# libvips/libvips

Measured on NVIDIA H100. Metric: Mpixels/s for thumbnail(4K->512,lanczos3), higher is better.
Workload: dtype u8

## Files before the change

### include/vb200.h

```cpp
#ifndef VB200_H
#define VB200_H

#include <stddef.h>
#include <stdint.h>

#ifdef __cplusplus
extern "C" {
#endif


typedef enum {
	VB200_FORMAT_UCHAR = 0,
	VB200_FORMAT_CHAR = 1,
	VB200_FORMAT_USHORT = 2,
	VB200_FORMAT_SHORT = 3,
	VB200_FORMAT_UINT = 4,
	VB200_FORMAT_INT = 5,
	VB200_FORMAT_FLOAT = 6,
	VB200_FORMAT_COMPLEX = 7,
	VB200_FORMAT_DOUBLE = 8,
	VB200_FORMAT_DPCOMPLEX = 9
} VB200BandFormat;

typedef enum {
// ... 135 lines not shown

typedef struct VB200ThumbnailPlan VB200ThumbnailPlan;

VB200ThumbnailPlan *vb200_thumbnail_plan_new(int width, int height, int bands, int band_format, int has_alpha,
	int target_width, int target_height, int size, int linear);
void vb200_thumbnail_plan_free(VB200ThumbnailPlan *plan);
int vb200_thumbnail_plan_output(const VB200ThumbnailPlan *plan, int *out_width, int *out_height);
int vb200_thumbnail_batch_device(VB200ThumbnailPlan *plan, const void *in, size_t in_frame_stride, void *out,
	size_t out_frame_stride, int n_frames);
int vb200_thumbnail_batch_host(VB200ThumbnailPlan *plan, const void *in, size_t in_frame_stride, void *out,
	size_t out_frame_stride, int n_frames);
int vb200_thumbnail_plan_set_sharpen(VB200ThumbnailPlan *plan, double sigma, double x1, double y2, double y3, double m1, double m2);
int vb200_thumbnail_plan_is_fused(const VB200ThumbnailPlan *plan);
size_t vb200_thumbnail_plan_bytes_per_frame(const VB200ThumbnailPlan *plan);
const char *vb200_thumbnail_plan_kernel(const VB200ThumbnailPlan *plan);

typedef struct {
	const void *input_profile;
	size_t input_len;
	const void *output_profile;
	size_t output_len;
	const void *builtin_rgb;
	size_t builtin_rgb_len;
	const void *builtin_grey;
	size_t builtin_grey_len;
	int intent;
} VB200ThumbnailIcc;

int vb200_thumbnail_plan_set_icc(VB200ThumbnailPlan *plan, const VB200ThumbnailIcc *icc);
int vb200_thumbnail_plan_output_bands(const VB200ThumbnailPlan *plan);
// ... 93 lines not shown
```

### libvips_b200/__init__.py

```python
import ctypes as C
import os

import numpy as np

_HERE = os.path.dirname(os.path.abspath(__file__))
_LIB_PATH = os.environ.get("VB200_LIB") or os.path.join(_HERE, "libvb200.so")
_lib = None

HOST, DEVICE = 0, 1

FORMATS = {np.dtype(np.uint8): 0, np.dtype(np.int8): 1, np.dtype(np.uint16): 2, np.dtype(np.int16): 3,
           np.dtype(np.uint32): 4, np.dtype(np.int32): 5, np.dtype(np.float32): 6, np.dtype(np.float64): 8}
DTYPES = {v: k for k, v in FORMATS.items()}
KERNELS = {"nearest": 0, "linear": 1, "cubic": 2, "mitchell": 3, "lanczos2": 4, "lanczos3": 5,
           "mks2013": 6, "mks2021": 7}
SIZES = {"both": 0, "up": 1, "down": 2, "force": 3}
PRECISIONS = {"integer": 0, "float": 1, "approximate": 2}
INTENTS = {"perceptual": 0, "relative": 1, "saturation": 2, "absolute": 3}
PCS = {"lab": 0, "xyz": 1}
INTERPRETATIONS = {"multiband": 0, "b-w": 1, "cmyk": 15, "xyz": 12, "lab": 13, "lch": 19, "labs": 21, "srgb": 22,
                   "yxy": 23, "rgb16": 25, "grey16": 26, "scrgb": 28, "hsv": 29}


class Error(Exception):
# ... 112 lines not shown
                                              C.c_size_t, C.c_size_t, PI, PI, PI]
        L.vb200_debug_jpeg_decode.argtypes = [C.c_void_p, C.c_size_t, C.c_int, C.c_void_p, C.c_size_t, PI, PI, PI]
        L.vb200_thumbnail_jpegshrink.argtypes = [C.c_int] * 5
        L.vb200_jpegsave_batch.argtypes = [C.c_void_p, C.c_int, C.c_size_t, C.c_size_t, C.c_int, C.c_int, C.c_int, C.c_int, C.c_int, C.c_int,
                                           C.c_void_p, C.c_int, C.c_size_t, C.POINTER(C.c_size_t)]
        L.vb200_thumbnail_buffer.argtypes = [C.c_void_p, C.c_size_t, IP, C.c_int, C.c_int, C.c_int]
        L.vb200_thumbnail_plan_run_jpeg.argtypes = [C.c_void_p, C.POINTER(C.c_void_p), C.POINTER(C.c_size_t), C.c_int, C.c_int,
                                                    C.c_void_p, C.c_int, C.c_size_t]
        L.vb200_thumbnail_plan_free.argtypes = [C.c_void_p]
        L.vb200_thumbnail_plan_output.argtypes = [C.c_void_p, C.POINTER(C.c_int), C.POINTER(C.c_int)]
        L.vb200_thumbnail_plan_bytes_per_frame.restype = C.c_size_t
        L.vb200_thumbnail_plan_bytes_per_frame.argtypes = [C.c_void_p]
        L.vb200_thumbnail_plan_is_fused.argtypes = [C.c_void_p]
        L.vb200_thumbnail_plan_kernel.restype = C.c_char_p
        L.vb200_thumbnail_plan_kernel.argtypes = [C.c_void_p]
        L.vb200_thumbnail_batch_device.argtypes = [C.c_void_p, C.c_void_p, C.c_size_t, C.c_void_p, C.c_size_t,
                                                   C.c_int]
        L.vb200_thumbnail_batch_host.argtypes = [C.c_void_p, C.c_void_p, C.c_size_t, C.c_void_p, C.c_size_t,
                                                 C.c_int]
        TI = C.POINTER(CThumbnailIcc)
        L.vb200_thumbnail_plan_set_icc.argtypes = [C.c_void_p, TI]
        L.vb200_thumbnail_plan_output_bands.argtypes = [C.c_void_p]
        L.vb200_thumbnail_batch_device_icc.argtypes = [C.c_void_p, C.c_void_p, C.c_size_t, C.c_void_p, C.c_size_t, C.c_int,
                                                       C.c_void_p, C.c_void_p]
        L.vb200_thumbnail_batch_host_icc.argtypes = L.vb200_thumbnail_batch_device_icc.argtypes
        L.vb200_thumbnail_image_icc.argtypes = [IP, IP, C.c_int, C.c_int, C.c_int, TI, C.c_char_p, C.c_size_t]
        L.vb200_thumbnail_buffer_icc.argtypes = [C.c_void_p, C.c_size_t, IP, C.c_int, C.c_int, C.c_int, TI]
        L.vb200_jpeg_icc_profile.argtypes = [C.c_char_p, C.c_size_t, C.c_void_p, C.c_size_t, C.POINTER(C.c_size_t)]
        L.vb200_debug_icc_select.argtypes = [TI, C.c_int, C.c_char_p, C.c_size_t, C.POINTER(C.c_int)]
        L.vb200_debug_icc_classify.argtypes = [C.c_char_p, C.c_size_t, C.c_int, C.c_int]
# ... 554 lines not shown
```

### libvips_b200/csrc/thumbnail_fused.cu

```cuda
#include <algorithm>
#include <climits>
#include <cmath>
#include <cstring>
#include <map>
#include <memory>
#include <mutex>
#include <vector>

#include <cuda.h>

#include "vb200_internal.h"

namespace vb200 {

namespace {

constexpr int kChunkRows = 8;
constexpr int kMaxThreads = 576;

struct FusedParams {
	int W, H;
	size_t in_bpl;
	int VS;
	int Hs;
// ... 10 lines not shown
	int TW;
	int RPC;
	int NT;
	int NEmax;
	int slots;
	int stage_pitch;
	int vgrid, hgrid;
	const int2 *vrow;
	const int2 *hcol;
	const int *vcoef;
	const int *hcoef;
	int nvsets, nhsets;
	const int2 *vchunk;
	const uint4 *vbfrag;
	int mma_rows;
	int premul;
	const unsigned char *opaque_hint;
	double max_alpha;
};

__device__ __forceinline__ int
dp2a_lo(unsigned coef, unsigned bytes, int acc)
{
	int d;
	asm("dp2a.lo.s32.u32 %0, %1, %2, %3;" : "=r"(d) : "r"(coef), "r"(bytes), "r"(acc));
	return d;
}

__device__ __forceinline__ int
dp2a_hi(unsigned coef, unsigned bytes, int acc)
// ... 1169 lines not shown
	int OW = 0, OH = 0;
	ReduceGeom gv{}, gh{};
	bool premul = false;
	bool fused = false;
	int device = -1;
	FusedParams fp{};
	void *tables = nullptr;
	size_t smem = 0;
	dim3 grid;
	bool tma_ok = false;
	int slots_tma = 0;
	size_t smem_tma = 0;
	bool tma3_ok = false;
	size_t smem_tma3 = 0;
	bool mma_ok = false;
	int mma_cols = 0, mma_cpt = 1, mma_tw = 0, mma_nt = 0, mma_nemax = 0;
	size_t smem_mma = 0;
	void *tables_mma = nullptr;
	static constexpr int kStreams = 3;
	cudaStream_t streams[kStreams] = {nullptr, nullptr, nullptr};
	void *stage_in[kStreams] = {nullptr, nullptr, nullptr};
	void *stage_out[kStreams] = {nullptr, nullptr, nullptr};
	cudaEvent_t drained[kStreams] = {nullptr, nullptr, nullptr};
	int stage_frames = 0;
	std::mutex pump_lock;
	std::mutex launch_lock;
	static constexpr int kHintSlots = 4;
	std::mutex hint_lock;
	int *hint_counts = nullptr;
	cudaEvent_t hint_done[kHintSlots] = {nullptr, nullptr, nullptr, nullptr};
	bool hint_pending[kHintSlots] = {false, false, false, false};
// ... 301 lines not shown
launch_mma_t(const char *domain, ThumbnailPlanImpl *pl, const FusedParams &fp, const void *in, size_t in_stride, void *out,
	size_t out_stride, int n, dim3 grid, cudaStream_t s)
{
	CUtensorMap tm;
	memset(&tm, 0, sizeof(tm));
	const int use_tmap = make_stage_tensor_map(&tm, in, fp.W, fp.H, fp.in_bpl, in_stride, n, (WCOLS + 8) / (WCOLS + 8 > 512 ? 2 : 1), 2 * VS) ? 1 : 0;
	constexpr bool CAN_OPQ = PREMUL && CPT == 2 && WCOLS > 448;
	for (int f0 = 0; f0 < n; f0 += 32768) {
		grid.z = std::min(32768, n - f0);
		FusedParams fpl = fp;
		void *hint = nullptr;
		bool use_opq = false;
		if (CAN_OPQ && opaque_hint_begin(domain, pl, fp, (const uint8_t *) in + (size_t) f0 * in_stride, in_stride, (int) grid.z, s, &hint, &use_opq))
			return -1;
		fpl.opaque_hint = (const unsigned char *) hint;
		int rc;
		if constexpr (CAN_OPQ)
			rc = use_opq ? launch_mma_k<VS, NP, PREMUL, HSQ, WCOLS, CPT, true>(domain, pl, fpl, tm, use_tmap, in, in_stride, out, out_stride, f0, grid, s)
						 : launch_mma_k<VS, NP, PREMUL, HSQ, WCOLS, CPT, false>(domain, pl, fpl, tm, use_tmap, in, in_stride, out, out_stride, f0, grid, s);
		else
			rc = launch_mma_k<VS, NP, PREMUL, HSQ, WCOLS, CPT, false>(domain, pl, fpl, tm, use_tmap, in, in_stride, out, out_stride, f0, grid, s);
		opaque_hint_end(pl, hint, (int) grid.z, s);
		if (rc)
			return rc;
	}
	return 0;
}

template <bool PREMUL, int WCOLS, int CPT>
int
launch_mma_w(const char *domain, ThumbnailPlanImpl *pl, const FusedParams &fp, const void *in, size_t is, void *out,
	size_t os, int n, dim3 grid, cudaStream_t s, bool *handled)
{
	*handled = true;
	const int np = fp.NPh == 6 || fp.NPh == 7 ? fp.NPh : 0;
#define V4(VS_, NP_, HS_) \
	if (fp.VS == VS_ && np == NP_ && fp.HS == HS_) \
// ... 4 lines not shown
	if constexpr (CPT == 2 && WCOLS > 448) {
		V4(3, 0, 3) V4(5, 0, 5) V4(6, 0, 6) V4(7, 0, 7)
		V4(2, 0, 3) V4(3, 0, 2) V4(3, 0, 4) V4(4, 0, 3) V4(4, 0, 5) V4(5, 0, 4) V4(5, 0, 6) V4(6, 0, 5)
		V4(6, 0, 7) V4(7, 0, 6) V4(7, 0, 8) V4(8, 0, 7)
	}
#undef V4
	*handled = false;
	return 0;
}

int
launch_mma(const char *domain, ThumbnailPlanImpl *pl, const void *in, size_t is, void *out, size_t os, int n,
	cudaStream_t s, bool *handled)
{
	FusedParams fp = pl->fp;
	fp.TW = pl->mma_tw;
	fp.NT = pl->mma_nt;
	fp.NEmax = pl->mma_nemax;
	const int K = fp.mma_rows;
	const int bands_x = (pl->OW + fp.TW - 1) / fp.TW;
	int rpc = ((pl->OH + K - 1) / K) * K;
	const int ctas = pl->mma_cols > 448 ? sm_count() : 2 * sm_count();
	while ((long long) bands_x * ((pl->OH + rpc - 1) / rpc) * n < ctas && rpc > 4 * K)
		rpc = ((rpc / 2 + K - 1) / K) * K;
	fp.RPC = rpc;
	const dim3 grid(bands_x, (pl->OH + rpc - 1) / rpc, 1);
	if (pl->mma_cols > 448)
		return pl->premul ? launch_mma_w<true, 768, 2>(domain, pl, fp, in, is, out, os, n, grid, s, handled)
						  : launch_mma_w<false, 768, 2>(domain, pl, fp, in, is, out, os, n, grid, s, handled);
	if (pl->mma_cpt == 1)
		return pl->premul ? launch_mma_w<true, VB200_V4_COLS, 1>(domain, pl, fp, in, is, out, os, n, grid, s, handled)
						  : launch_mma_w<false, VB200_V4_COLS, 1>(domain, pl, fp, in, is, out, os, n, grid, s, handled);
	return pl->premul ? launch_mma_w<true, VB200_V4_COLS, 2>(domain, pl, fp, in, is, out, os, n, grid, s, handled)
					  : launch_mma_w<false, VB200_V4_COLS, 2>(domain, pl, fp, in, is, out, os, n, grid, s, handled);
}
// ... 49 lines not shown
	if (pl->gv.int_shrink > 1) {
		tile_w = tg.tile_width;
		tile_h = tg.tile_height;
	}
	else {
		tile_w = pl->OW;
		tile_h = tg.fatstrip_height;
	}
	int rect_h = tile_h;
	if (pl->gh.int_shrink > 1)
		rect_h = std::min(rect_h, tg.fatstrip_height);
	build_axis_table(tv, pl->OH, pl->gv.residual, pl->gv.offset, pl->gv.n_point, VB200_KERNEL_LANCZOS3, rect_h);
	build_axis_table(th, pl->OW, pl->gh.residual, pl->gh.offset, pl->gh.n_point, VB200_KERNEL_LANCZOS3, tile_w);
}

int
plan_build_fused(const char *domain, ThumbnailPlanImpl *pl)
{
	AxisTable tv, th;
	plan_axis_tables(pl, tv, th);

	auto build_sets = [](const AxisTable &t, int count, int grid, PairSets &sets, std::vector<int2> &idx) {
		sets = PairSets();
		sets.NP = (t.n_point + 2) / 2;
		idx.resize(count);
		for (int i = 0; i < count; i++) {
			const int rel = t.first[i] - grid;
			idx[i].x = rel >> 1;
			idx[i].y = sets.get(t, t.phase[i], rel & 1);
		}
		sets.trim();
	};
	PairSets sv, shh;
	std::vector<int2> vrow, hcol;
	int vgrid = 0, hgrid = 0;
	{
		PairSets alt;
		std::vector<int2> alt_idx;
		build_sets(tv, pl->OH, 0, sv, vrow);
		build_sets(tv, pl->OH, 1, alt, alt_idx);
		if (alt.NP < sv.NP) {
			sv = alt;
			vrow = alt_idx;
			vgrid = 1;
		}
		build_sets(th, pl->OW, 0, shh, hcol);
		build_sets(th, pl->OW, 1, alt, alt_idx);
		if (alt.NP < shh.NP) {
			shh = alt;
			hcol = alt_idx;
			hgrid = 1;
		}
	}

	FusedParams &fp = pl->fp;
	fp.W = pl->W;
	fp.H = pl->H;
	fp.in_bpl = (size_t) pl->W * 4;
	fp.VS = pl->gv.int_shrink;
	fp.Hs = pl->gv.shrunk_size;
	fp.vembed = tv.embed;
	fp.NPv = sv.NP;
	fp.vgrid = vgrid;
	fp.hgrid = hgrid;
	fp.vmul8 = (unsigned) (((1LL << 32) / (256LL * fp.VS)) << 8);
	fp.vshift = -1;
	fp.accmul = 1;
	for (int sft = 0; sft < 9; sft++)
// ... 110 lines not shown
		if (ok) {
			memcpy(vchunk.data(), vchunk_flat.data(), vchunk.size() * sizeof(int2));
			memcpy(bfrag.data(), bfrag_flat.data(), bfrag.size() * sizeof(uint4));
		}
		const char *ev = getenv("VB200_V4_COLS");
		const int wcols = ev && atoi(ev) <= 448 && vpow2 && hpow2 ? VB200_V4_COLS : 768;
		const int warp_cols = hpow2 ? 0 : 2 * (32 / fp.HS) * fp.HS;
		pl->mma_cpt = wcols > 448 || (getenv("VB200_V4_CPT") && atoi(getenv("VB200_V4_CPT")) == 2) ? 2 : 1;
		const int pitch = (wcols + 8) * 4;
		auto column_of = [&](int E0, int tt) {
			const int e = E0 + tt / fp.HS;
			const int k = tt % fp.HS;
			const int sc = std::max(0, std::min(e - fp.hembed, fp.Ws - 1));
			return std::min(sc * fp.HS + k, fp.W - 1);
		};
		int tw4 = 0, nemax4 = 0;
		long best_cost = LONG_MAX;
		const int cols_per_warp = warp_cols ? warp_cols : 32 * pl->mma_cpt;
		const int col_budget = warp_cols ? (wcols / 64) * warp_cols : wcols;
		for (int tw = std::min(pl->OW, 256); tw >= 2 && ok; tw--) {
			int worst = 0, max_cols = 0;
			long cost = 0;
			for (int xa = 0; xa < pl->OW; xa += tw) {
				const int xb = std::min(xa + tw, pl->OW);
				const int E0 = 2 * hcol[xa].x + hgrid;
				const int ne = 2 * (hcol[xb - 1].x + fp.NPh - hcol[xa].x);
				const int c_lo = column_of(E0, 0) & ~3;
				const int c_hi = std::min(fp.W, (column_of(E0, ne * fp.HS - 1) + 4) & ~3);
				worst = std::max(worst, ne);
				max_cols = std::max(max_cols, c_hi - c_lo);
				cost += (ne * fp.HS + cols_per_warp - 1) / cols_per_warp + 1;
			}
			if (worst * fp.HS <= col_budget && max_cols * 4 <= pitch && cost < best_cost) {
				best_cost = cost;
				tw4 = tw;
				nemax4 = worst;
			}
		}
		if (ok && tw4 > 0) {
			pl->mma_cols = wcols;
			pl->mma_tw = tw4;
			pl->mma_nemax = nemax4;
			pl->mma_nt = warp_cols ? std::max(64, ((nemax4 * fp.HS + warp_cols - 1) / warp_cols) * 32)
								   : std::max(64, ((nemax4 * fp.HS / pl->mma_cpt + 31) / 32) * 32);
			const int stages = fp.VS <= 2 ? 2 * VB200_V4_STAGES
				: (fp.VS >= 7 ? VB200_V4_STAGES / 2 : (fp.VS >= 5 ? (3 * VB200_V4_STAGES) / 4 : VB200_V4_STAGES));
			const int logical_cols = warp_cols ? (pl->mma_nt / 32) * warp_cols : pl->mma_nt * pl->mma_cpt;
			const int nbox = wcols + 8 > 512 ? 2 : 1;
			const size_t box_bytes = ((size_t) 2 * fp.VS * (pitch / nbox) + 127) & ~(size_t) 127;
			pl->smem_mma = (size_t) stages * nbox * box_bytes + (2 * stages + 4) * 8 +
				(size_t) kV4Quads * ((size_t) pl->mma_nt * pl->mma_cpt * 16 + 16) +
				(size_t) 2 * kV4Rows * ((logical_cols / fp.HS + 1) / 2) * 8 +
				(size_t) (fp.nhsets * fp.NPh + 256) * 4;
			const size_t n_ch = vchunk.size() * sizeof(int2), n_bf = bfrag.size() * sizeof(uint4);
			if (pl->smem_mma <= (wcols > 448 ? 226 : 113) * 1024) {
				VB200_CUDA(domain, cudaMalloc(&pl->tables_mma, n_bf + n_ch));
				VB200_CUDA(domain, cudaMemcpy(pl->tables_mma, bfrag.data(), n_bf, cudaMemcpyHostToDevice));
				VB200_CUDA(domain, cudaMemcpy((char *) pl->tables_mma + n_bf, vchunk.data(), n_ch, cudaMemcpyHostToDevice));
				fp.vbfrag = (const uint4 *) pl->tables_mma;
				fp.vchunk = (const int2 *) ((char *) pl->tables_mma + n_bf);
				pl->mma_ok = true;
			}
		}
	}

	const size_t n_vrow = vrow.size() * sizeof(int2), n_hcol = hcol.size() * sizeof(int2);
	const size_t n_vc = sv.coef.size() * 4, n_hc = shh.coef.size() * 4;
	std::vector<char> host(n_vrow + n_hcol + n_vc + n_hc);
	memcpy(&host[0], vrow.data(), n_vrow);
	memcpy(&host[n_vrow], hcol.data(), n_hcol);
	memcpy(&host[n_vrow + n_hcol], sv.coef.data(), n_vc);
	memcpy(&host[n_vrow + n_hcol + n_vc], shh.coef.data(), n_hc);
	VB200_CUDA(domain, cudaMalloc(&pl->tables, host.size()));
	VB200_CUDA(domain, cudaMemcpy(pl->tables, host.data(), host.size(), cudaMemcpyHostToDevice));
	char *b = (char *) pl->tables;
// ... 29 lines not shown
__global__ void __launch_bounds__(256)
rgbx_compact_kernel(const uint8_t *__restrict__ in, size_t in_stride, uint8_t *__restrict__ out, size_t out_stride, size_t pixels)
{
	const size_t i = (size_t) blockIdx.x * blockDim.x + threadIdx.x;
	if (i >= pixels)
		return;
	const unsigned px = __ldg((const unsigned *) (in + (size_t) blockIdx.y * in_stride) + i);
	uint8_t *q = out + (size_t) blockIdx.y * out_stride + i * 3;
	q[0] = (uint8_t) px;
	q[1] = (uint8_t) (px >> 8);
	q[2] = (uint8_t) (px >> 16);
}

}

int
thumbnail_plan_init(const char *domain, ThumbnailPlanImpl *pl)
{
	if (pl->fmt != VB200_FORMAT_UCHAR) {
		error(domain, "only uchar frames are on the batched device path");
		return -1;
	}
	thumbnail_shrink(pl->W, pl->H, pl->target_w, pl->target_h, pl->size, &pl->hshrink, &pl->vshrink);
	if (pl->linear && (pl->bands < 3 || pl->hshrink < 1.0 || pl->vshrink < 1.0)) {
		error(domain, pl->bands < 3 ? "linear thumbnails on the device path need an 8-bit image with 3+ bands"
									: "upsizing is not on the device path yet");
		return -1;
	}
	if (pl->hshrink < 1.0 || pl->vshrink < 1.0) {
		const double hscale = std::max(1.0 / pl->hshrink, 1.0 / pl->W);
		const double vscale = std::max(1.0 / pl->vshrink, 1.0 / pl->H);
		if (hscale < 1.0 || vscale < 1.0) {
			error(domain, "mixed up/down resize is not on the device path");
			return -1;
		}
		const double rw = (hscale > 1.0 ? hscale : 1.0) * pl->W, rh = (vscale > 1.0 ? vscale : 1.0) * pl->H;
		pl->OW = (int) (rw > 0 ? rw + 0.5 : rw - 0.5);
		pl->OH = (int) (rh > 0 ? rh + 0.5 : rh - 0.5);
		pl->premul = pl->has_alpha && pl->hshrink != 1.0 && pl->vshrink != 1.0;
		pl->fused = false;
		return 0;
	}
	double hscale = std::max(1.0 / pl->hshrink, 1.0 / pl->W);
	double vscale = std::max(1.0 / pl->vshrink, 1.0 / pl->H);
	const double vs = vscale < 1.0 ? 1.0 / vscale : 1.0;
	const double hs = hscale < 1.0 ? 1.0 / hscale : 1.0;
	pl->gv = ReduceGeom{pl->H, pl->H, 1, pl->H, 0, 1.0, 0.0};
	pl->gh = ReduceGeom{pl->W, pl->W, 1, pl->W, 0, 1.0, 0.0};
	if (vs > 1.0 && reduce_geometry(domain, pl->H, vs, VB200_KERNEL_LANCZOS3, 2.0, &pl->gv))
		return -1;
	if (hs > 1.0 && reduce_geometry(domain, pl->W, hs, VB200_KERNEL_LANCZOS3, 2.0, &pl->gh))
		return -1;
	pl->OW = pl->gh.out_size;
	pl->OH = pl->gv.out_size;
	pl->premul = pl->has_alpha && pl->hshrink != 1.0 && pl->vshrink != 1.0;

	pl->fused = false;
	if (pl->linear) {
		AxisTable tv, th;
		if (pl->gv.n_point > 0 && pl->gh.n_point > 0) {
			plan_axis_tables(pl, tv, th);
			if (linear_thumb_new(domain, pl->W, pl->H, pl->bands, pl->premul, pl->gv, pl->gh, tv, th, &pl->lin) < 0)
				return -1;
		}
		pl->fused = pl->lin != nullptr;
		return 0;
	}
	pl->rgb_expand = pl->bands == 3 && ((size_t) pl->W * pl->H) % 4 == 0 && getenv("VB200_NO_RGB_EXPAND") == nullptr;
	if ((pl->bands == 4 || pl->rgb_expand) && pl->gv.n_point > 0 && pl->gh.n_point > 0) {
// ... 453 lines not shown
	if (pl.linear)
		return "linear_v_kernel + linear_h_kernel";
	const FusedParams &fp = pl.fp;
	const int nph = fp.NPh == 6 || fp.NPh == 7 ? fp.NPh : 0;
	const bool v4 = pl.mma_ok;
	if (v4)
		snprintf(name, sizeof(name), "thumbnail_fused_mma_kernel<VS=%d,NP=%d,%s,HS=%d,cols=%d,cpt=%d>", fp.VS, nph,
			pl.premul ? "premul" : "plain", fp.HS, pl.mma_cols, pl.mma_cpt);
	else if (pl.tma3_ok)
		snprintf(name, sizeof(name), "thumbnail_fused_tma3_kernel<VS=%d,%s,HS=%d>", fp.VS, pl.premul ? "premul" : "plain", fp.HS);
	else if (pl.tma_ok)
		snprintf(name, sizeof(name), "thumbnail_fused_tma_kernel<VS=%d,%s>", fp.VS, pl.premul ? "premul" : "plain");
	else
		snprintf(name, sizeof(name), "thumbnail_fused_kernel<VS=%d,%s>", fp.VS, pl.premul ? "premul" : "plain");
	return name;
}

extern "C" int
vb200_thumbnail_batch_device(VB200ThumbnailPlan *plan, const void *in, size_t in_frame_stride, void *out,
	size_t out_frame_stride, int n_frames)
{
	return vb200_thumbnail_batch_device_icc(plan, in, in_frame_stride, out, out_frame_stride, n_frames, nullptr, nullptr);
}

extern "C" int
vb200_thumbnail_batch_device_icc(VB200ThumbnailPlan *plan, const void *in, size_t in_frame_stride, void *out,
	size_t out_frame_stride, int n_frames, const void *const *embedded, const size_t *embedded_lens)
{
	const char *domain = "thumbnail_batch_device";
	if (!plan || !in || !out) {
// ... 380 lines not shown
```

### libvips_b200/csrc/thumbnail_fused_mma.cuh

```cuda

constexpr int kV4Rows = 8;
constexpr int kV4Quads = 8;

#ifndef VB200_V4_COLS
#define VB200_V4_COLS 384
#endif
#ifndef VB200_V4_STAGES
#define VB200_V4_STAGES 4
#endif
#ifndef VB200_V4_NH768
#define VB200_V4_NH768 3
#endif
#ifndef VB200_V4_MMA_UNROLL
#define VB200_V4_MMA_UNROLL 2
#endif
#ifndef VB200_V4_HPOLL_NS
#define VB200_V4_HPOLL_NS 0
#endif
#ifndef VB200_V4_PPOLL_NS
#define VB200_V4_PPOLL_NS 0
#endif
#ifndef VB200_V4_VPOLL_NS
#define VB200_V4_VPOLL_NS 0
#endif
#ifndef VB200_V4_EPOLL_NS
#define VB200_V4_EPOLL_NS 0
// ... 53 lines not shown
__device__ __forceinline__ void
mma_u8u8(int (&d)[4], const unsigned (&a)[4], unsigned b0, unsigned b1)
{
	asm volatile("mma.sync.aligned.m16n8k32.row.col.s32.u8.u8.s32 {%0,%1,%2,%3}, {%4,%5,%6,%7}, {%8,%9}, {%0,%1,%2,%3};"
				 : "+r"(d[0]), "+r"(d[1]), "+r"(d[2]), "+r"(d[3])
				 : "r"(a[0]), "r"(a[1]), "r"(a[2]), "r"(a[3]), "r"(b0), "r"(b1));
}

__device__ __forceinline__ int
v4_finish(int hi, int lo, int k20)
{
	const int v = __mulhi(hi * 256 + lo, k20);
	return max(0, min(v, 255));
}

template <int VS, int NP, bool PREMUL, int HSQ, int WCOLS, int CPT, bool OPQ = false>
__global__ void __launch_bounds__(WCOLS / CPT + 32 * V4HWarpsW<WCOLS, CPT>::value + 32, WCOLS <= 448 ? 2 : 1)
thumbnail_fused_mma_kernel(const __grid_constant__ FusedParams P, const __grid_constant__ CUtensorMap tmap, int use_tmap,
	const uint8_t *__restrict__ in, size_t in_frame_stride, uint8_t *__restrict__ out, size_t out_frame_stride, int frame0)
{
	extern __shared__ __align__(128) unsigned char smem_raw[];

	constexpr int KM = kV4Rows;
	const int K = P.mma_rows;
	constexpr int S = V4Stages<VS>::value;
	constexpr int NH = V4HWarpsW<WCOLS, CPT>::value;
	constexpr int kMmaUnroll = VB200_V4_MMA_UNROLL;
	constexpr int NBOX = WCOLS + 8 > 512 ? 2 : 1;
	constexpr int BOXW = (WCOLS + 8) / NBOX;
	constexpr int PITCH = BOXW * 4;
	constexpr int NPR = NP > 0 ? NP : 1;
	constexpr int HSHIFT = HSQ == 2 ? 1 : HSQ == 4 ? 2 : 3;
	constexpr bool VPOW2 = (VS & (VS - 1)) == 0;
	constexpr bool HPOW2 = V4Group<HSQ>::pow2;
	constexpr int G = V4Group<HSQ>::value;
	static_assert(HPOW2 || CPT == 2, "non-power-of-two horizontal boxes are built for two columns per thread");
	constexpr int rows_per_stage = 2 * VS;
	constexpr unsigned box_bytes = ((unsigned) rows_per_stage * PITCH + 127u) & ~127u;
	constexpr unsigned stage_bytes = NBOX * box_bytes;

	const int NT = P.NT;
	const int NC = NT * CPT;
	const int t = threadIdx.x;
	const int NPh = NP > 0 ? NP : P.NPh;
	const int LC = HPOW2 ? NC : (NT / 32) * 2 * G;
	const int shs = (LC / HSQ + 1) / 2;
// ... 4 lines not shown
	unsigned char *quadbuf = (unsigned char *) (bars + 2 * S + 4);
	uint2 *sh = (uint2 *) (quadbuf + (size_t) kV4Quads * QS);
	int *hcoef = (int *) (sh + (size_t) 2 * KM * shs);
	int *uscale = hcoef + P.nhsets * P.NPh;

	const unsigned stages_s = smem_addr(stages);
	const unsigned full_s = smem_addr(bars);
	const unsigned empty_s = full_s + 8u * S;
	const unsigned shfull_s = empty_s + 8u * S;
	const unsigned shempty_s = shfull_s + 16u;

	for (int i = t; i < P.nhsets * P.NPh; i += blockDim.x)
		hcoef[i] = P.hcoef[i];
	if (PREMUL)
		for (int i = t; i < 256; i += blockDim.x)
			uscale[i] = i == 0 ? 0 : (int) __ddiv_rn(__dmul_rn(256.0, 255.0), (double) i);

	const int xa = blockIdx.x * P.TW;
	const int xb = min(xa + P.TW, P.OW);
	const int y_begin = blockIdx.y * P.RPC;
	const int y_end = min(y_begin + P.RPC, P.OH);
	const int frame = frame0 + blockIdx.z;
	const uint8_t *fin = in + (size_t) frame * in_frame_stride;
	uint8_t *fout = out + (size_t) frame * out_frame_stride;

	const int pair_h0 = __ldg(&P.hcol[xa]).x;
	const int E0 = 2 * pair_h0 + P.hgrid;
	const int NE = 2 * (__ldg(&P.hcol[xb - 1]).x + P.NPh - pair_h0);

	auto column_of = [&](int tt) {
		const int e = E0 + tt / HSQ;
		const int k = tt - (tt / HSQ) * HSQ;
		const int sc = max(0, min(e - P.hembed, P.Ws - 1));
		return min(sc * HSQ + k, P.W - 1);
	};
	const int c_lo = column_of(0) & ~3;
	const int c_hi = min(P.W, (column_of(NE * HSQ - 1) + 4) & ~3);
	const unsigned row_bytes = (unsigned) (c_hi - c_lo) * 4u;
	const int chunk0 = y_begin / K;
	const int q_first = __ldg(&P.vchunk[chunk0]).x;
	const int NTa = HPOW2 ? min(NT, ((NE * HSQ + 32 * CPT - 1) / (32 * CPT)) * 32) : min(NT, ((NE * HSQ + 2 * G - 1) / (2 * G)) * 32);

	if (t == 0) {
// ... 54 lines not shown
					}
				}
				if (++s == S) {
					s = 0;
					phase ^= 1u;
				}
			}
			pdone = max(pdone, P1 + 1);
		}
		return;
	}

	if (t >= NT) {
		const int ht = t - NT;
		const int lane = ht & 31;
		const int bw = xb - xa;
		int chunk = 0;
		for (int ya = y_begin; ya < y_end; ya += K, chunk++) {
			const int yb = min(ya + K, y_end);
			const int rows = yb - ya;
			const int buf = chunk & 1;
			const uint2 *shb = sh + (size_t) buf * KM * shs;
			if (VB200_V4_HPOLL_NS)
				mbar_wait_poll(shfull_s + 8u * buf, (unsigned) (chunk >> 1) & 1u, VB200_V4_HPOLL_NS);
			else
				mbar_wait(shfull_s + 8u * buf, (unsigned) (chunk >> 1) & 1u);
			for (int idx = ht; idx < rows * bw; idx += 32 * NH) {
				const int k = fast_div(idx, bw);
				const int x = xa + (idx - k * bw);
				const int2 hc = __ldg(&P.hcol[x]);
				const uint2 *win = shb + k * shs + (hc.x - pair_h0);
				const int *cfp = hcoef + hc.y * NPh;
				int r = VB200_INTERPOLATE_SCALE >> 1, g = r, b = r, a = r;
				if (NP > 0) {
#pragma unroll
					for (int kk = 0; kk < NPR; kk++) {
						const uint2 w = win[kk];
						const unsigned c = (unsigned) cfp[kk];
						r = dp2a_lo(c, w.x, r);
						b = dp2a_hi(c, w.x, b);
						g = dp2a_lo(c, w.y, g);
						a = dp2a_hi(c, w.y, a);
					}
				}
				else
					for (int kk = 0; kk < NPh; kk++) {
						const uint2 w = win[kk];
						const unsigned c = (unsigned) cfp[kk];
						r = dp2a_lo(c, w.x, r);
						b = dp2a_hi(c, w.x, b);
						g = dp2a_lo(c, w.y, g);
						a = dp2a_hi(c, w.y, a);
					}
				r = max(0, min(r >> VB200_INTERPOLATE_SHIFT, 255));
				g = max(0, min(g >> VB200_INTERPOLATE_SHIFT, 255));
				b = max(0, min(b >> VB200_INTERPOLATE_SHIFT, 255));
				a = max(0, min(a >> VB200_INTERPOLATE_SHIFT, 255));
				if (PREMUL) {
					const int sc = uscale[a];
					r = ((r * sc + 128) >> 8) & 0xff;
					g = ((g * sc + 128) >> 8) & 0xff;
					b = ((b * sc + 128) >> 8) & 0xff;
				}
				*(unsigned *) (fout + (size_t) (ya + k) * P.out_bpl + (size_t) x * 4) =
					(unsigned) r | ((unsigned) g << 8) | ((unsigned) b << 16) | ((unsigned) a << 24);
			}
			__syncwarp();
			if (lane == 0)
				mbar_arrive(shempty_s + 8u * buf);
		}
		return;
	}

	if (t >= NTa)
		return;
	const int lane_ = t & 31;
	const int tt0 = HPOW2 ? t * CPT
						  : (t >> 5) * 2 * G + (lane_ >> 4) * G + min((lane_ & 15) * 2, G - 2);
	const int my_c = column_of(min(tt0, NE * HSQ - CPT)) - c_lo;
	const unsigned char *my_cols = stages + (size_t) (my_c / BOXW) * box_bytes + (size_t) (my_c % BOXW) * 4u;
// ... 246 lines not shown
							d[0] = (unsigned char) __umulhi((unsigned) (bsum[0] + HSQ / 2), hmul8);
							d[(size_t) shs * 8] = (unsigned char) __umulhi((unsigned) (bsum[1] + HSQ / 2), hmul8);
							bsum[0] = bsum[1] = 0;
							bcnt = 0;
							bidx++;
						}
					}
				}
			}
		}
		__syncwarp();
		if (lane0)
			mbar_arrive(shfull_s + 8u * buf);
	}
}
```

Baseline: 685,400.

## Partition horizontal bands by input pairs and fix seam columns in a follow-up kernel

Replaces the fixed-output-width tiling of the MMA fused thumbnail kernel with a band partition over input pairs, so bands no longer overlap their input windows. Output columns whose filter window straddles a band boundary are finished by a new seam kernel that reads edge pairs saved to a scratch buffer. It also cuts the default horizontal-warp count for the 768-column variant. In exchange it adds a per-batch device allocation, an extra kernel launch and seam scratch writes.

```diff
diff --git a/include/vb200.h b/include/vb200.h
--- a/include/vb200.h
+++ b/include/vb200.h
@@ -173,6 +173,8 @@
 int vb200_thumbnail_plan_is_fused(const VB200ThumbnailPlan *plan);
 size_t vb200_thumbnail_plan_bytes_per_frame(const VB200ThumbnailPlan *plan);
 const char *vb200_thumbnail_plan_kernel(const VB200ThumbnailPlan *plan);
+int vb200_debug_thumbnail_bands(int width, int height, int target_width, int target_height, int size, int *info, int *bands,
+	int cap, int *first_pair);
 
 typedef struct {
 	const void *input_profile;
diff --git a/libvips_b200/__init__.py b/libvips_b200/__init__.py
--- a/libvips_b200/__init__.py
+++ b/libvips_b200/__init__.py
@@ -150,6 +150,8 @@
         L.vb200_thumbnail_plan_is_fused.argtypes = [C.c_void_p]
         L.vb200_thumbnail_plan_kernel.restype = C.c_char_p
         L.vb200_thumbnail_plan_kernel.argtypes = [C.c_void_p]
+        L.vb200_debug_thumbnail_bands.argtypes = [C.c_int, C.c_int, C.c_int, C.c_int, C.c_int, C.c_void_p, C.c_void_p,
+                                                  C.c_int, C.c_void_p]
         L.vb200_thumbnail_batch_device.argtypes = [C.c_void_p, C.c_void_p, C.c_size_t, C.c_void_p, C.c_size_t,
                                                    C.c_int]
         L.vb200_thumbnail_batch_host.argtypes = [C.c_void_p, C.c_void_p, C.c_size_t, C.c_void_p, C.c_size_t,
diff --git a/libvips_b200/csrc/thumbnail_fused.cu b/libvips_b200/csrc/thumbnail_fused.cu
--- a/libvips_b200/csrc/thumbnail_fused.cu
+++ b/libvips_b200/csrc/thumbnail_fused.cu
@@ -48,6 +48,10 @@
 	const int2 *vchunk;
 	const uint4 *vbfrag;
 	int mma_rows;
+	const int4 *vband;
+	const int2 *seamcol;
+	int nbands, nseamcols;
+	uint2 *seam;
 	int premul;
 	const unsigned char *opaque_hint;
 	double max_alpha;
@@ -1247,7 +1251,7 @@
 	bool tma3_ok = false;
 	size_t smem_tma3 = 0;
 	bool mma_ok = false;
-	int mma_cols = 0, mma_cpt = 1, mma_tw = 0, mma_nt = 0, mma_nemax = 0;
+	int mma_cols = 0, mma_cpt = 1, mma_nt = 0, mma_nemax = 0;
 	size_t smem_mma = 0;
 	void *tables_mma = nullptr;
 	static constexpr int kStreams = 3;
@@ -1579,6 +1583,12 @@
 		if (CAN_OPQ && opaque_hint_begin(domain, pl, fp, (const uint8_t *) in + (size_t) f0 * in_stride, in_stride, (int) grid.z, s, &hint, &use_opq))
 			return -1;
 		fpl.opaque_hint = (const unsigned char *) hint;
+		void *seam = nullptr;
+		if (fp.nseamcols > 0 && dev_alloc(domain, &seam, (size_t) grid.z * fp.nbands * 2 * fp.OH * fp.NPh * sizeof(uint2), s)) {
+			opaque_hint_end(pl, hint, (int) grid.z, s);
+			return -1;
+		}
+		fpl.seam = (uint2 *) seam;
 		int rc;
 		if constexpr (CAN_OPQ)
 			rc = use_opq ? launch_mma_k<VS, NP, PREMUL, HSQ, WCOLS, CPT, true>(domain, pl, fpl, tm, use_tmap, in, in_stride, out, out_stride, f0, grid, s)
@@ -1586,6 +1596,18 @@
 		else
 			rc = launch_mma_k<VS, NP, PREMUL, HSQ, WCOLS, CPT, false>(domain, pl, fpl, tm, use_tmap, in, in_stride, out, out_stride, f0, grid, s);
 		opaque_hint_end(pl, hint, (int) grid.z, s);
+		if (!rc && seam) {
+			const int items = fp.nseamcols * fp.OH;
+			const dim3 sgrid((unsigned) std::max(1, std::min((items + 2047) / 2048, 64)), grid.z, 1);
+			thumbnail_seam_kernel<NP, PREMUL><<<sgrid, 256, 0, s>>>(fpl, (uint8_t *) out, out_stride, f0);
+			const cudaError_t e = cudaGetLastError();
+			if (e != cudaSuccess)
+				rc = cuda_fail(domain, e, "thumbnail_seam_kernel launch");
+			else
+				count_launch();
+		}
+		if (seam)
+			dev_free(seam, s);
 		if (rc)
 			return rc;
 	}
@@ -1620,11 +1642,10 @@
 	cudaStream_t s, bool *handled)
 {
 	FusedParams fp = pl->fp;
-	fp.TW = pl->mma_tw;
 	fp.NT = pl->mma_nt;
 	fp.NEmax = pl->mma_nemax;
 	const int K = fp.mma_rows;
-	const int bands_x = (pl->OW + fp.TW - 1) / fp.TW;
+	const int bands_x = fp.nbands;
 	int rpc = ((pl->OH + K - 1) / K) * K;
 	const int ctas = pl->mma_cols > 448 ? sm_count() : 2 * sm_count();
 	while ((long long) bands_x * ((pl->OH + rpc - 1) / rpc) * n < ctas && rpc > 4 * K)
@@ -1704,44 +1725,96 @@
 	build_axis_table(th, pl->OW, pl->gh.residual, pl->gh.offset, pl->gh.n_point, VB200_KERNEL_LANCZOS3, tile_w);
 }
 
+void
+build_pair_sets(const AxisTable &t, int count, PairSets &sets, std::vector<int2> &idx, int &grid)
+{
+	auto build = [&](int g, PairSets &s, std::vector<int2> &ix) {
+		s = PairSets();
+		s.NP = (t.n_point + 2) / 2;
+		ix.resize(count);
+		for (int i = 0; i < count; i++) {
+			const int rel = t.first[i] - g;
+			ix[i].x = rel >> 1;
+			ix[i].y = s.get(t, t.phase[i], rel & 1);
+		}
+		s.trim();
+	};
+	PairSets alt;
+	std::vector<int2> alt_idx;
+	build(0, sets, idx);
+	build(1, alt, alt_idx);
+	grid = 0;
+	if (alt.NP < sets.NP) {
+		sets = alt;
+		idx = alt_idx;
+		grid = 1;
+	}
+}
+
+int
+v4_max_pairs(int HS, int wcols)
+{
+	const bool hpow2 = HS == 2 || HS == 4 || HS == 8;
+	const int vwarps = wcols > 448 ? wcols / 64 - 1 : wcols / 64;
+	const int col_budget = vwarps * (hpow2 ? 64 : 2 * (32 / HS) * HS);
+	return col_budget / (2 * HS);
+}
+
+
+std::vector<int4>
+v4_band_partition(const std::vector<int2> &hcol, int NPh, int hgrid, int hembed, int HS, int max_pairs)
+{
+	const int OW = (int) hcol.size();
+	const int lo = hcol[0].x, hi = hcol[OW - 1].x + NPh, T = hi - lo;
+	std::vector<int> q;
+	if (T <= max_pairs)
+		q = {lo, hi};
+	for (int nb = std::max(2, (T + max_pairs - 1) / max_pairs); q.empty() && nb * NPh <= T; nb++)
+		for (int align = 64; align >= 1 && q.empty(); align /= 2) {
+			q = {lo};
+			for (int b = 1; b < nb && !q.empty(); b++) {
+				const int qmin = std::max(q.back() + NPh, hi - (nb - b) * max_pairs);
+				const int qmax = std::min(q.back() + max_pairs, hi - (nb - b) * NPh);
+				const double even = lo + (double) T * b / nb;
+				int best = INT_MIN;
+				for (int c = qmin; c <= qmax; c++)
+					if (((2 * c + hgrid - hembed) * HS) % align == 0 && (best == INT_MIN || fabs(c - even) < fabs(best - even)))
+						best = c;
+				if (best == INT_MIN)
+					q.clear();
+				else
+					q.push_back(best);
+			}
+			if (!q.empty())
+				q.push_back(hi);
+		}
+	std::vector<int4> bands;
+	for (size_t b = 0; b + 1 < q.size(); b++) {
+		int4 v;
+		v.x = q[b];
+		v.y = q[b + 1];
+		v.z = 0;
+		while (v.z < OW && hcol[v.z].x < v.x)
+			v.z++;
+		v.w = v.z;
+		while (v.w < OW && hcol[v.w].x + NPh <= v.y)
+			v.w++;
+		bands.push_back(v);
+	}
+	return bands;
+}
+
 int
 plan_build_fused(const char *domain, ThumbnailPlanImpl *pl)
 {
 	AxisTable tv, th;
 	plan_axis_tables(pl, tv, th);
 
-	auto build_sets = [](const AxisTable &t, int count, int grid, PairSets &sets, std::vector<int2> &idx) {
-		sets = PairSets();
-		sets.NP = (t.n_point + 2) / 2;
-		idx.resize(count);
-		for (int i = 0; i < count; i++) {
-			const int rel = t.first[i] - grid;
-			idx[i].x = rel >> 1;
-			idx[i].y = sets.get(t, t.phase[i], rel & 1);
-		}
-		sets.trim();
-	};
 	PairSets sv, shh;
 	std::vector<int2> vrow, hcol;
 	int vgrid = 0, hgrid = 0;
-	{
-		PairSets alt;
-		std::vector<int2> alt_idx;
-		build_sets(tv, pl->OH, 0, sv, vrow);
-		build_sets(tv, pl->OH, 1, alt, alt_idx);
-		if (alt.NP < sv.NP) {
-			sv = alt;
-			vrow = alt_idx;
-			vgrid = 1;
-		}
-		build_sets(th, pl->OW, 0, shh, hcol);
-		build_sets(th, pl->OW, 1, alt, alt_idx);
-		if (alt.NP < shh.NP) {
-			shh = alt;
-			hcol = alt_idx;
-			hgrid = 1;
-		}
-	}
+	build_pair_sets(tv, pl->OH, sv, vrow, vgrid);
+	build_pair_sets(th, pl->OW, shh, hcol, hgrid);
 
 	FusedParams &fp = pl->fp;
 	fp.W = pl->W;
@@ -1882,32 +1955,23 @@
 			const int sc = std::max(0, std::min(e - fp.hembed, fp.Ws - 1));
 			return std::min(sc * fp.HS + k, fp.W - 1);
 		};
-		int tw4 = 0, nemax4 = 0;
-		long best_cost = LONG_MAX;
-		const int cols_per_warp = warp_cols ? warp_cols : 32 * pl->mma_cpt;
-		const int col_budget = warp_cols ? (wcols / 64) * warp_cols : wcols;
-		for (int tw = std::min(pl->OW, 256); tw >= 2 && ok; tw--) {
-			int worst = 0, max_cols = 0;
-			long cost = 0;
-			for (int xa = 0; xa < pl->OW; xa += tw) {
-				const int xb = std::min(xa + tw, pl->OW);
-				const int E0 = 2 * hcol[xa].x + hgrid;
-				const int ne = 2 * (hcol[xb - 1].x + fp.NPh - hcol[xa].x);
-				const int c_lo = column_of(E0, 0) & ~3;
-				const int c_hi = std::min(fp.W, (column_of(E0, ne * fp.HS - 1) + 4) & ~3);
-				worst = std::max(worst, ne);
-				max_cols = std::max(max_cols, c_hi - c_lo);
-				cost += (ne * fp.HS + cols_per_warp - 1) / cols_per_warp + 1;
-			}
-			if (worst * fp.HS <= col_budget && max_cols * 4 <= pitch && cost < best_cost) {
-				best_cost = cost;
-				tw4 = tw;
-				nemax4 = worst;
-			}
-		}
-		if (ok && tw4 > 0) {
+		const std::vector<int4> bands = ok ? v4_band_partition(hcol, fp.NPh, hgrid, fp.hembed, fp.HS, v4_max_pairs(fp.HS, wcols))
+										   : std::vector<int4>();
+		int nemax4 = 0, max_cols = 0;
+		std::vector<int2> seamcol;
+		for (size_t b = 0; b < bands.size(); b++) {
+			const int E0 = 2 * bands[b].x + hgrid;
+			const int ne = 2 * (bands[b].y - bands[b].x);
+			const int c_lo = column_of(E0, 0) & ~3;
+			const int c_hi = std::min(fp.W, (column_of(E0, ne * fp.HS - 1) + 4) & ~3);
+			nemax4 = std::max(nemax4, ne);
+			max_cols = std::max(max_cols, c_hi - c_lo);
+			if (b + 1 < bands.size())
+				for (int x = bands[b].w; x < bands[b + 1].z; x++)
+					seamcol.push_back(make_int2(x, (int) b));
+		}
+		if (ok && !bands.empty() && max_cols * 4 <= pitch) {
 			pl->mma_cols = wcols;
-			pl->mma_tw = tw4;
 			pl->mma_nemax = nemax4;
 			pl->mma_nt = warp_cols ? std::max(64, ((nemax4 * fp.HS + warp_cols - 1) / warp_cols) * 32)
 								   : std::max(64, ((nemax4 * fp.HS / pl->mma_cpt + 31) / 32) * 32);
@@ -1921,12 +1985,22 @@
 				(size_t) 2 * kV4Rows * ((logical_cols / fp.HS + 1) / 2) * 8 +
 				(size_t) (fp.nhsets * fp.NPh + 256) * 4;
 			const size_t n_ch = vchunk.size() * sizeof(int2), n_bf = bfrag.size() * sizeof(uint4);
+			const size_t n_bd = bands.size() * sizeof(int4), n_sc = seamcol.size() * sizeof(int2);
 			if (pl->smem_mma <= (wcols > 448 ? 226 : 113) * 1024) {
-				VB200_CUDA(domain, cudaMalloc(&pl->tables_mma, n_bf + n_ch));
-				VB200_CUDA(domain, cudaMemcpy(pl->tables_mma, bfrag.data(), n_bf, cudaMemcpyHostToDevice));
-				VB200_CUDA(domain, cudaMemcpy((char *) pl->tables_mma + n_bf, vchunk.data(), n_ch, cudaMemcpyHostToDevice));
-				fp.vbfrag = (const uint4 *) pl->tables_mma;
-				fp.vchunk = (const int2 *) ((char *) pl->tables_mma + n_bf);
+				char *tb;
+				VB200_CUDA(domain, cudaMalloc(&pl->tables_mma, n_bf + n_bd + n_ch + n_sc));
+				tb = (char *) pl->tables_mma;
+				VB200_CUDA(domain, cudaMemcpy(tb, bfrag.data(), n_bf, cudaMemcpyHostToDevice));
+				VB200_CUDA(domain, cudaMemcpy(tb + n_bf, bands.data(), n_bd, cudaMemcpyHostToDevice));
+				VB200_CUDA(domain, cudaMemcpy(tb + n_bf + n_bd, vchunk.data(), n_ch, cudaMemcpyHostToDevice));
+				if (n_sc)
+					VB200_CUDA(domain, cudaMemcpy(tb + n_bf + n_bd + n_ch, seamcol.data(), n_sc, cudaMemcpyHostToDevice));
+				fp.vbfrag = (const uint4 *) tb;
+				fp.vband = (const int4 *) (tb + n_bf);
+				fp.vchunk = (const int2 *) (tb + n_bf + n_bd);
+				fp.seamcol = (const int2 *) (tb + n_bf + n_bd + n_ch);
+				fp.nbands = (int) bands.size();
+				fp.nseamcols = (int) seamcol.size();
 				pl->mma_ok = true;
 			}
 		}
@@ -1986,33 +2060,9 @@
 
 }
 
-int
-thumbnail_plan_init(const char *domain, ThumbnailPlanImpl *pl)
-{
-	if (pl->fmt != VB200_FORMAT_UCHAR) {
-		error(domain, "only uchar frames are on the batched device path");
-		return -1;
-	}
-	thumbnail_shrink(pl->W, pl->H, pl->target_w, pl->target_h, pl->size, &pl->hshrink, &pl->vshrink);
-	if (pl->linear && (pl->bands < 3 || pl->hshrink < 1.0 || pl->vshrink < 1.0)) {
-		error(domain, pl->bands < 3 ? "linear thumbnails on the device path need an 8-bit image with 3+ bands"
-									: "upsizing is not on the device path yet");
-		return -1;
-	}
-	if (pl->hshrink < 1.0 || pl->vshrink < 1.0) {
-		const double hscale = std::max(1.0 / pl->hshrink, 1.0 / pl->W);
-		const double vscale = std::max(1.0 / pl->vshrink, 1.0 / pl->H);
-		if (hscale < 1.0 || vscale < 1.0) {
-			error(domain, "mixed up/down resize is not on the device path");
-			return -1;
-		}
-		const double rw = (hscale > 1.0 ? hscale : 1.0) * pl->W, rh = (vscale > 1.0 ? vscale : 1.0) * pl->H;
-		pl->OW = (int) (rw > 0 ? rw + 0.5 : rw - 0.5);
-		pl->OH = (int) (rh > 0 ? rh + 0.5 : rh - 0.5);
-		pl->premul = pl->has_alpha && pl->hshrink != 1.0 && pl->vshrink != 1.0;
-		pl->fused = false;
-		return 0;
-	}
+static int
+plan_reduce_geometry(const char *domain, ThumbnailPlanImpl *pl)
+{
 	double hscale = std::max(1.0 / pl->hshrink, 1.0 / pl->W);
 	double vscale = std::max(1.0 / pl->vshrink, 1.0 / pl->H);
 	const double vs = vscale < 1.0 ? 1.0 / vscale : 1.0;
@@ -2025,6 +2075,38 @@
 		return -1;
 	pl->OW = pl->gh.out_size;
 	pl->OH = pl->gv.out_size;
+	return 0;
+}
+
+int
+thumbnail_plan_init(const char *domain, ThumbnailPlanImpl *pl)
+{
+	if (pl->fmt != VB200_FORMAT_UCHAR) {
+		error(domain, "only uchar frames are on the batched device path");
+		return -1;
+	}
+	thumbnail_shrink(pl->W, pl->H, pl->target_w, pl->target_h, pl->size, &pl->hshrink, &pl->vshrink);
+	if (pl->linear && (pl->bands < 3 || pl->hshrink < 1.0 || pl->vshrink < 1.0)) {
+		error(domain, pl->bands < 3 ? "linear thumbnails on the device path need an 8-bit image with 3+ bands"
+									: "upsizing is not on the device path yet");
+		return -1;
+	}
+	if (pl->hshrink < 1.0 || pl->vshrink < 1.0) {
+		const double hscale = std::max(1.0 / pl->hshrink, 1.0 / pl->W);
+		const double vscale = std::max(1.0 / pl->vshrink, 1.0 / pl->H);
+		if (hscale < 1.0 || vscale < 1.0) {
+			error(domain, "mixed up/down resize is not on the device path");
+			return -1;
+		}
+		const double rw = (hscale > 1.0 ? hscale : 1.0) * pl->W, rh = (vscale > 1.0 ? vscale : 1.0) * pl->H;
+		pl->OW = (int) (rw > 0 ? rw + 0.5 : rw - 0.5);
+		pl->OH = (int) (rh > 0 ? rh + 0.5 : rh - 0.5);
+		pl->premul = pl->has_alpha && pl->hshrink != 1.0 && pl->vshrink != 1.0;
+		pl->fused = false;
+		return 0;
+	}
+	if (plan_reduce_geometry(domain, pl))
+		return -1;
 	pl->premul = pl->has_alpha && pl->hshrink != 1.0 && pl->vshrink != 1.0;
 
 	pl->fused = false;
@@ -2508,6 +2590,48 @@
 	else
 		snprintf(name, sizeof(name), "thumbnail_fused_kernel<VS=%d,%s>", fp.VS, pl.premul ? "premul" : "plain");
 	return name;
+}
+
+extern "C" int
+vb200_debug_thumbnail_bands(int width, int height, int target_width, int target_height, int size, int *info, int *bands,
+	int cap, int *first_pair)
+{
+	const char *domain = "vb200_debug_thumbnail_bands";
+	ThumbnailPlanImpl pl;
+	pl.W = width;
+	pl.H = height;
+	pl.target_w = target_width;
+	pl.target_h = target_height > 0 ? target_height : target_width;
+	pl.size = size;
+	if (width < 1 || height < 1 || target_width < 1)
+		return -1;
+	thumbnail_shrink(pl.W, pl.H, pl.target_w, pl.target_h, pl.size, &pl.hshrink, &pl.vshrink);
+	if (pl.hshrink < 1.0 || pl.vshrink < 1.0 || plan_reduce_geometry(domain, &pl))
+		return -1;
+	if (pl.gv.n_point <= 0 || pl.gh.n_point <= 0)
+		return 0;
+	AxisTable tv, th;
+	plan_axis_tables(&pl, tv, th);
+	PairSets shh;
+	std::vector<int2> hcol;
+	int hgrid = 0;
+	build_pair_sets(th, pl.OW, shh, hcol, hgrid);
+	const int HS = pl.gh.int_shrink;
+	const std::vector<int4> part = v4_band_partition(hcol, shh.NP, hgrid, th.embed, HS, v4_max_pairs(HS, 768));
+	const int v[7] = {pl.OW, shh.NP, HS, hgrid, th.embed, pl.gh.shrunk_size, v4_max_pairs(HS, 768)};
+	memcpy(info, v, sizeof(v));
+	if ((int) part.size() > cap)
+		return -1;
+	for (size_t b = 0; b < part.size(); b++) {
+		bands[4 * b] = part[b].x;
+		bands[4 * b + 1] = part[b].y;
+		bands[4 * b + 2] = part[b].z;
+		bands[4 * b + 3] = part[b].w;
+	}
+	if (first_pair)
+		for (int x = 0; x < pl.OW; x++)
+			first_pair[x] = hcol[x].x;
+	return (int) part.size();
 }
 
 extern "C" int
diff --git a/libvips_b200/csrc/thumbnail_fused_mma.cuh b/libvips_b200/csrc/thumbnail_fused_mma.cuh
--- a/libvips_b200/csrc/thumbnail_fused_mma.cuh
+++ b/libvips_b200/csrc/thumbnail_fused_mma.cuh
@@ -9,7 +9,7 @@
 #define VB200_V4_STAGES 4
 #endif
 #ifndef VB200_V4_NH768
-#define VB200_V4_NH768 3
+#define VB200_V4_NH768 1
 #endif
 #ifndef VB200_V4_MMA_UNROLL
 #define VB200_V4_MMA_UNROLL 2
@@ -93,6 +93,51 @@
 	return max(0, min(v, 255));
 }
 
+template <int NP, bool PREMUL, class Win>
+__device__ __forceinline__ unsigned
+reduceh_pixel(const Win &win, const int *cfp, int NPh, const int *uscale)
+{
+	constexpr int NPR = NP > 0 ? NP : 1;
+	int r = VB200_INTERPOLATE_SCALE >> 1, g = r, b = r, a = r;
+	if (NP > 0) {
+#pragma unroll
+		for (int kk = 0; kk < NPR; kk++) {
+			const uint2 w = win(kk);
+			const unsigned c = (unsigned) cfp[kk];
+			r = dp2a_lo(c, w.x, r);
+			b = dp2a_hi(c, w.x, b);
+			g = dp2a_lo(c, w.y, g);
+			a = dp2a_hi(c, w.y, a);
+		}
+	}
+	else
+		for (int kk = 0; kk < NPh; kk++) {
+			const uint2 w = win(kk);
+			const unsigned c = (unsigned) cfp[kk];
+			r = dp2a_lo(c, w.x, r);
+			b = dp2a_hi(c, w.x, b);
+			g = dp2a_lo(c, w.y, g);
+			a = dp2a_hi(c, w.y, a);
+		}
+	r = max(0, min(r >> VB200_INTERPOLATE_SHIFT, 255));
+	g = max(0, min(g >> VB200_INTERPOLATE_SHIFT, 255));
+	b = max(0, min(b >> VB200_INTERPOLATE_SHIFT, 255));
+	a = max(0, min(a >> VB200_INTERPOLATE_SHIFT, 255));
+	if (PREMUL) {
+		const int sc = uscale[a];
+		r = ((r * sc + 128) >> 8) & 0xff;
+		g = ((g * sc + 128) >> 8) & 0xff;
+		b = ((b * sc + 128) >> 8) & 0xff;
+	}
+	return (unsigned) r | ((unsigned) g << 8) | ((unsigned) b << 16) | ((unsigned) a << 24);
+}
+
+__device__ __forceinline__ int
+unpremultiply_scale(int a)
+{
+	return a == 0 ? 0 : (int) __ddiv_rn(__dmul_rn(256.0, 255.0), (double) a);
+}
+
 template <int VS, int NP, bool PREMUL, int HSQ, int WCOLS, int CPT, bool OPQ = false>
 __global__ void __launch_bounds__(WCOLS / CPT + 32 * V4HWarpsW<WCOLS, CPT>::value + 32, WCOLS <= 448 ? 2 : 1)
 thumbnail_fused_mma_kernel(const __grid_constant__ FusedParams P, const __grid_constant__ CUtensorMap tmap, int use_tmap,
@@ -108,7 +153,6 @@
 	constexpr int NBOX = WCOLS + 8 > 512 ? 2 : 1;
 	constexpr int BOXW = (WCOLS + 8) / NBOX;
 	constexpr int PITCH = BOXW * 4;
-	constexpr int NPR = NP > 0 ? NP : 1;
 	constexpr int HSHIFT = HSQ == 2 ? 1 : HSQ == 4 ? 2 : 3;
 	constexpr bool VPOW2 = (VS & (VS - 1)) == 0;
 	constexpr bool HPOW2 = V4Group<HSQ>::pow2;
@@ -143,19 +187,20 @@
 		hcoef[i] = P.hcoef[i];
 	if (PREMUL)
 		for (int i = t; i < 256; i += blockDim.x)
-			uscale[i] = i == 0 ? 0 : (int) __ddiv_rn(__dmul_rn(256.0, 255.0), (double) i);
-
-	const int xa = blockIdx.x * P.TW;
-	const int xb = min(xa + P.TW, P.OW);
+			uscale[i] = unpremultiply_scale(i);
+
+	const int4 band = __ldg(&P.vband[blockIdx.x]);
+	const int xa = band.z;
+	const int xb = band.w;
 	const int y_begin = blockIdx.y * P.RPC;
 	const int y_end = min(y_begin + P.RPC, P.OH);
 	const int frame = frame0 + blockIdx.z;
 	const uint8_t *fin = in + (size_t) frame * in_frame_stride;
 	uint8_t *fout = out + (size_t) frame * out_frame_stride;
 
-	const int pair_h0 = __ldg(&P.hcol[xa]).x;
+	const int pair_h0 = band.x;
 	const int E0 = 2 * pair_h0 + P.hgrid;
-	const int NE = 2 * (__ldg(&P.hcol[xb - 1]).x + P.NPh - pair_h0);
+	const int NE = 2 * (band.y - pair_h0);
 
 	auto column_of = [&](int tt) {
 		const int e = E0 + tt / HSQ;
@@ -240,7 +285,8 @@
 	if (t >= NT) {
 		const int ht = t - NT;
 		const int lane = ht & 31;
-		const int bw = xb - xa;
+		const int bw = max(0, xb - xa);
+		uint2 *seam = P.seam ? P.seam + ((size_t) blockIdx.z * gridDim.x + blockIdx.x) * 2 * P.OH * NPh : nullptr;
 		int chunk = 0;
 		for (int ya = y_begin; ya < y_end; ya += K, chunk++) {
 			const int yb = min(ya + K, y_end);
@@ -256,40 +302,18 @@
 				const int x = xa + (idx - k * bw);
 				const int2 hc = __ldg(&P.hcol[x]);
 				const uint2 *win = shb + k * shs + (hc.x - pair_h0);
-				const int *cfp = hcoef + hc.y * NPh;
-				int r = VB200_INTERPOLATE_SCALE >> 1, g = r, b = r, a = r;
-				if (NP > 0) {
-#pragma unroll
-					for (int kk = 0; kk < NPR; kk++) {
-						const uint2 w = win[kk];
-						const unsigned c = (unsigned) cfp[kk];
-						r = dp2a_lo(c, w.x, r);
-						b = dp2a_hi(c, w.x, b);
-						g = dp2a_lo(c, w.y, g);
-						a = dp2a_hi(c, w.y, a);
-					}
-				}
-				else
-					for (int kk = 0; kk < NPh; kk++) {
-						const uint2 w = win[kk];
-						const unsigned c = (unsigned) cfp[kk];
-						r = dp2a_lo(c, w.x, r);
-						b = dp2a_hi(c, w.x, b);
-						g = dp2a_lo(c, w.y, g);
-						a = dp2a_hi(c, w.y, a);
-					}
-				r = max(0, min(r >> VB200_INTERPOLATE_SHIFT, 255));
-				g = max(0, min(g >> VB200_INTERPOLATE_SHIFT, 255));
-				b = max(0, min(b >> VB200_INTERPOLATE_SHIFT, 255));
-				a = max(0, min(a >> VB200_INTERPOLATE_SHIFT, 255));
-				if (PREMUL) {
-					const int sc = uscale[a];
-					r = ((r * sc + 128) >> 8) & 0xff;
-					g = ((g * sc + 128) >> 8) & 0xff;
-					b = ((b * sc + 128) >> 8) & 0xff;
-				}
 				*(unsigned *) (fout + (size_t) (ya + k) * P.out_bpl + (size_t) x * 4) =
-					(unsigned) r | ((unsigned) g << 8) | ((unsigned) b << 16) | ((unsigned) a << 24);
+					reduceh_pixel<NP, PREMUL>([&](int kk) { return win[kk]; }, hcoef + hc.y * NPh, NPh, uscale);
+			}
+			if (seam) {
+				const int half = NE / 2 - NPh;
+				for (int idx = ht; idx < rows * 2 * NPh; idx += 32 * NH) {
+					const int k = fast_div(idx, 2 * NPh);
+					const int j = idx - k * 2 * NPh;
+					const int side = j >= NPh ? 1 : 0;
+					const int jj = j - side * NPh;
+					seam[((size_t) side * P.OH + ya + k) * NPh + jj] = shb[k * shs + side * half + jj];
+				}
 			}
 			__syncwarp();
 			if (lane == 0)
@@ -566,3 +590,33 @@
 			mbar_arrive(shfull_s + 8u * buf);
 	}
 }
+
+template <int NP, bool PREMUL>
+__global__ void __launch_bounds__(256)
+thumbnail_seam_kernel(const __grid_constant__ FusedParams P, uint8_t *__restrict__ out, size_t out_frame_stride, int frame0)
+{
+	__shared__ int uscale[256];
+	if (PREMUL)
+		for (int i = threadIdx.x; i < 256; i += blockDim.x)
+			uscale[i] = unpremultiply_scale(i);
+	__syncthreads();
+	const int NPh = NP > 0 ? NP : P.NPh;
+	const int M = P.nseamcols;
+	const uint2 *fseam = P.seam + (size_t) blockIdx.y * P.nbands * 2 * P.OH * NPh;
+	uint8_t *fout = out + (size_t) (frame0 + blockIdx.y) * out_frame_stride;
+	for (int i = blockIdx.x * blockDim.x + threadIdx.x; i < M * P.OH; i += gridDim.x * blockDim.x) {
+		const int y = i / M;
+		const int2 sc = __ldg(&P.seamcol[i - y * M]);
+		const int q = __ldg(&P.vband[sc.y]).y;
+		const uint2 *left = fseam + ((size_t) (2 * sc.y + 1) * P.OH + y) * NPh;
+		const uint2 *right = fseam + ((size_t) (2 * sc.y + 2) * P.OH + y) * NPh;
+		const int2 hc = __ldg(&P.hcol[sc.x]);
+		const int off = hc.x - (q - NPh);
+		*(unsigned *) (fout + (size_t) y * P.out_bpl + (size_t) sc.x * 4) = reduceh_pixel<NP, PREMUL>(
+			[&](int kk) {
+				const int j = off + kk;
+				return j < NPh ? __ldg(left + j) : __ldg(right + j - NPh);
+			},
+			P.hcoef + hc.y * NPh, NPh, uscale);
+	}
+}
```

After: 703,200 (median of 6 runs). 2.6% higher.
